# OnurBasci/TransformerBasedNavierStokeSolver

Measured on AMD Instinct MI355X. Metric: ns64_train_samples_per_s, higher is better.
Workload: dtype f32

## Files before the change

transformerbasednavierstokesolver_amd/csrc/pa2d_gemm.hip:

```cpp
#include "pa2d_gemm_common.h"
#include <string.h>


static Pa2dEnv read_env() {
    auto is = [](const char* n, const char* pre) { const char* e = getenv(n); return e && strncmp(e, pre, strlen(pre)) == 0; };
    auto num = [](const char* n, int dflt) { const char* e = getenv(n); return (e && e[0]) ? atoi(e) : dflt; };
    Pa2dEnv v;
    v.conv_halo = is("PA2D_CONV_HALO", "o") ? 0 : (is("PA2D_CONV_HALO", "f") ? 2 : 1);
    v.mc_big_off = is("PA2D_MC_BIG", "o") ? 1 : 0;
    v.kc_bk16 = num("PA2D_KC_BK", 0) == 16 ? 1 : 0;
    v.mc_bk = num("PA2D_MC_BK", 16) == 32 ? 32 : 16;
    v.mc_splits = num("PA2D_MC_SPLITS", 0);
    v.mcb_splits = num("PA2D_MCB_SPLITS", 0);
    v.lin_dw_split = is("PA2D_LIN_DW_SPLIT", "of") ? 0 : 1;
    v.lin_panel = is("PA2D_LIN_PANEL", "of") ? 0 : 1;
    v.lin_rowpanel = is("PA2D_LIN_ROWPANEL", "of") ? 0 : 1;
    v.lin_small_split = is("PA2D_LIN_SMALL_SPLIT", "of") ? 0 : 1;
    v.conv_mfma16 = num("PA2D_CONV_MFMA", 16) == 32 ? 0 : 1;
    v.mc_mfma16 = num("PA2D_MC_MFMA", 16) == 32 ? 0 : 1;
    v.split_big = num("PA2D_SPLIT_BIG", 1);
    v.slice_map = is("PA2D_SLICE_MAP", "l") ? 0 : 1;
    v.default_engine = is("PA2D_GEMM", "f") ? 0 : (is("PA2D_GEMM", "b") ? 2 : 1);
    return v;
}
static Pa2dEnv g_env = read_env();
const Pa2dEnv& pa2d_env() { return g_env; }
static int kc_bk(bool im2col, int Cin) {
    if (im2col && pa2d_env().kc_bk16) return 16;
    return (!im2col || (Cin % 32) == 0) ? 32 : 16;
}
KCTile kc_tile(int M, int N, bool im2col, int Cin) {
    const int tiles_m = ceil_div(M, 128);
    const long long t128 = (long long)tiles_m * ceil_div(N, 128);
    const long long t12864 = (long long)tiles_m * ceil_div(N, 64);
    const int bk = kc_bk(im2col, Cin);
    if (N > 64 && t128 >= 384) return {128, 128, bk};
    if (t12864 >= 384 || M <= 64) return {128, 64, bk};
    return {64, 64, bk};
}
bool use_split(int engine, int N, bool im2col, int Cin) {
    const int m = engine;
    if (m == 1) return im2col && N > 64 && (Cin % 32) == 0;
    if (m == 2) return N > 64 && (!im2col || (Cin % 32) == 0);
    return false;
}

int launch_kc(const KCParams& p_in, bool im2col, hipStream_t st, hipEvent_t ev0, hipEvent_t ev1) {
    KCParams p = p_in;
    if (!engine_ok(p.engine)) return PA2D_ERR_ARG;
    if (p.M <= 0 || p.N <= 0 || p.K <= 0) return PA2D_OK;
    if (!p.bias2) p.bias_split = 0x7fffffff;
    {
// ... 18 lines not shown
        if (p.wsrc) {
            rc = launch_pack_weight_image(p.wsrc, p.wsn, p.wsk, p.wimg, p.N, p.K, st);
            if (rc) return rc;
        }
        KCParams pp = p;
        pp.M = p.M - p.M % 128;
        rc = launch_kc_rowpanel(pp, p.wimg, st);
        if (!rc && pp.M < p.M) {
            KCParams pt = p_in;
            pt.wimg = nullptr;
            pt.M = p.M - pp.M;
            pt.A = p.A + (size_t)pp.M * p.lda;
            pt.C = p.C + (size_t)pp.M * p.ldc;
            if (p.res) pt.res = p.res + (size_t)pp.M * p.ldres;
            if (p.aux) pt.aux = p.aux + (size_t)pp.M * p.ldaux;
            rc = launch_kc(pt, false, st);
        }
    } else if (panel_applies(p, im2col)) {
        KCParams pp = p;
        pp.M = p.M - p.M % 256;
        rc = launch_kc_panel(pp, st);
        if (!rc && pp.M < p.M) {
            KCParams pt = p_in;
            const size_t ea = p.io_bf16 ? 2 : 4, es = p.io_bf16 ? 2 : 4;
            pt.M = p.M - pp.M;
            pt.A = (const float*)((const char*)p.A + (size_t)pp.M * p.lda * ea);
            pt.C = (float*)((char*)p.C + (size_t)pp.M * p.ldc * es);
            if (p.res) pt.res = (const float*)((const char*)p.res + (size_t)pp.M * p.ldres * es);
            if (p.aux) pt.aux = (float*)((char*)p.aux + (size_t)pp.M * p.ldaux * es);
            rc = launch_kc(pt, false, st);
        }
    } else if (p.io_bf16 || use_split(p.engine, p.N, im2col, p.Cin)) rc = launch_kc_split(p, im2col, st);
    else if (kc_split_small_applies(p, im2col)) rc = launch_kc_split_small(p, st);
    else rc = launch_kc_f32(p, im2col, kc_tile(p.M, p.N, im2col, p.Cin), st);
    if (rc) return rc;
    if (ev1 && hipEventRecord(ev1, st) != hipSuccess) return PA2D_ERR_ARG;
    return PA2D_OK;
}

template <int TAPS>
__global__ void repack_kernel(const float* __restrict__ w0, const float* __restrict__ w1, float* __restrict__ dst,
                              int mode, int N, int K, int C, int Cin, int NK) {
    const long long idx = (long long)blockIdx.x * blockDim.x + threadIdx.x;
    if (mode == 0) {
        if (idx >= (long long)N * K) return;
        const int n = (int)(idx % N), k = (int)(idx / N);
        dst[idx] = w0[(size_t)n * K + k];
    } else if (mode == 1) {
        if (idx >= (long long)NK * C * TAPS * Cin) return;
        const int CH = K;
        const int c16 = (int)(idx % CH);
        const int tap = (int)((idx / CH) % TAPS);
        const int cic = (int)((idx / (TAPS * CH)) % (Cin / CH));
        const int co = (int)(idx / ((long long)Cin * TAPS));
        const int ci = cic * CH + c16;
        const float* src = co < C ? w0 : w1;
        dst[idx] = src[((size_t)(co % C) * Cin + ci) * TAPS + tap];
    } else {
        if (idx >= (long long)NK * C * TAPS * Cin) return;
        const int CH = K;
        const int c16 = (int)(idx % CH);
        const int tap = (int)((idx / CH) % TAPS);
        const int cic = (int)((idx / (TAPS * CH)) % (NK * C / CH));
        const int ci = (int)(idx / ((long long)NK * C * TAPS));
        const int co = cic * CH + c16;
        const float* src = co < C ? w0 : w1;
// ... 62 lines not shown
                           const void* wimg, void* ws, size_t ws_bytes, int M, int N, int K, int act, int engine,
                           hipStream_t st) {
    KCParams p = dense_fwd_params(x, ldx, w, ldw, bias, res, ldres, y, ldy, pre, ldpre, M, N, K, act, engine, false);
    const size_t img = rowpanel_image_bytes(N, K, engine);
    if (img && wimg) p.wimg = const_cast<void*>(wimg);
    else if (ws && img && ws_bytes >= img) { p.wimg = ws; p.wsrc = w; p.wsn = ldw; p.wsk = 1; }
    return launch_kc(p, false, st);
}

int pa2d_gemm_bwd_data(const float* dy, long long lddy, const float* w, long long ldw, const float* pre,
                       long long ldpre, int act, float* dx, long long lddx, const void* wimg, void* ws, size_t ws_bytes, int M,
                       int N, int K, int engine, hipStream_t st) {
    if (ldw != K) return PA2D_ERR_ARG;
    if (N & 3) return PA2D_ERR_ARG;
    if (M <= 0) return PA2D_OK;
    if (ws_bytes < (size_t)N * K * sizeof(float)) return PA2D_ERR_WORKSPACE;
    float* const wt_ws = (float*)ws;
    KCParams p = dense_bwd_data_params(dy, lddy, wt_ws, pre, ldpre, act, dx, lddx, M, N, K, engine, false);
    const size_t img = rowpanel_image_bytes(K, N, engine);
    if (img && wimg) p.wimg = const_cast<void*>(wimg);
    else if (img && ws_bytes >= (size_t)N * K * sizeof(float) + img) {
        p.wimg = (char*)ws + (size_t)N * K * sizeof(float); p.wsrc = w; p.wsn = 1; p.wsk = ldw;
    }
    if (!(p.wimg && rowpanel_applies(p) && (M % 128) == 0)) {
        const int rc = launch_repack(w, nullptr, wt_ws, 0, N, K, 0, 0, st);
        if (rc) return rc;
    }
    return launch_kc(p, false, st);
}

size_t pa2d_gemm_bwd_weight_workspace(int M, int N, int K, int engine) {
    (void)engine;
    const MCPlan pl = plan_mc(N, K, M);
    return (pl.slab_floats + (size_t)pl.splits * N) * sizeof(float);
}

int pa2d_gemm_bwd_weight(const float* dy, long long lddy, const float* x, long long ldx, float* dw, float* db,
                         void* ws, size_t ws_bytes, int M, int N, int K, int accumulate, int engine, hipStream_t st) {
    if (!engine_ok(engine)) return PA2D_ERR_ARG;
    if (M <= 0) {
        if (accumulate) return PA2D_OK;
        const int rz = pa2d_zero(dw, sizeof(float) * N * K, st);
        return rz ? rz : pa2d_zero(db, sizeof(float) * N, st);
    }
    if (ws_bytes < pa2d_gemm_bwd_weight_workspace(M, N, K, engine)) return PA2D_ERR_WORKSPACE;
    const MCPlan pl = plan_mc(N, K, M);
    float* cs = db ? (float*)ws + pl.slab_floats : nullptr;
    const bool bfk = (engine == 1 || engine == 2) && pl.big && mc_f32src_applies(N, K, M, lddy, ldx);
    int rc = bfk ? launch_mc_f32src(dy, lddy, N, x, ldx, K, M, (float*)ws, pl, engine == 2 ? 1 : 3, cs, st)
                 : launch_mc(dy, lddy, N, x, ldx, K, M, false, 0, 0, 0, (float*)ws, pl, engine, st, cs);
    if (rc) return rc;
    rc = launch_reduce((const float*)ws, pl.splits, (long long)N * K, dw, nullptr, 0, 0, 0, st, accumulate);
    if (rc) return rc;
    if (db) rc = launch_reduce(cs, pl.splits, N, db, nullptr, 0, 0, 0, st, accumulate);
    return rc;
}


int pa2d_gemm_bias_act_fwd_bf16(const void* x, long long ldx, const float* w, long long ldw, const float* bias,
                                const void* res, long long ldres, void* y, long long ldy, void* pre, long long ldpre,
                                int M, int N, int K, int act, hipStream_t st) {
    return launch_kc(dense_fwd_params(x, ldx, w, ldw, bias, res, ldres, y, ldy, pre, ldpre, M, N, K, act, 2, true), false, st);
}

int pa2d_gemm_bwd_data_bf16(const void* dy, long long lddy, const float* w, long long ldw, const void* pre,
                            long long ldpre, int act, void* dx, long long lddx, float* wt_ws, int M, int N, int K,
                            hipStream_t st) {
    if (ldw != K) return PA2D_ERR_ARG;
    if (N & 3) return PA2D_ERR_ARG;
    if (M <= 0) return PA2D_OK;
    int rc = launch_repack(w, nullptr, wt_ws, 0, N, K, 0, 0, st);
    if (rc) return rc;
    return launch_kc(dense_bwd_data_params(dy, lddy, wt_ws, pre, ldpre, act, dx, lddx, M, N, K, 2, true), false, st);
}

size_t pa2d_gemm_bwd_weight_workspace_bf16(int M, int N, int K) {
    const MCPlan pl = plan_mc_planes_big(N, K, M);
    size_t a = pl.slab_floats, b = (size_t)colsum_blocks(M) * N;
// ... 24 lines not shown
```

transformerbasednavierstokesolver_amd/csrc/pa2d_gemm_common.h:

```cpp
#pragma once
#include "pa2d_internal.h"
#include "pa2d_bf16_split.h"
#include <stdlib.h>

#define EPI_ACT 1
#define EPI_STORE_PRE 2
#define EPI_MUL_DACT 4

struct KCParams {
    const float* A; long long lda;
    const float* B; long long ldb;
    float* C; long long ldc;
    const float* bias;
    const float* bias2; int bias_split;
    int depth;
    const float* res; long long ldres;
    float* aux; long long ldaux;
    int M, N, K;
    int act, epi;
    int H, W, Cin;
    unsigned a_bytes, b_bytes;
    unsigned c_bytes, res_bytes, aux_bytes;
    int apre;
    int engine;
// ... 104 lines not shown
bool kc_split_small_applies(const KCParams& p, bool im2col);
int launch_kc_split_small(const KCParams& p, hipStream_t st);
size_t planes_bytes(long long rows, int C, int NT);
int launch_split_planes(const float* src, long long ld, void* dst, long long rows, int C, int NT, hipStream_t st);
int launch_repack_split(const float* w0, const float* w1, void* dst, int bwd, int NT, int C, int Cin, hipStream_t st,
                        int taps = 9);
bool panel_applies(const KCParams& p, bool im2col);
int launch_kc_panel(const KCParams& p, hipStream_t st);
size_t rowpanel_image_bytes(int N, int K, int engine);
bool rowpanel_applies(const KCParams& p);
int launch_pack_weight_image(const float* w, long long sn, long long sk, void* img, int N, int K, hipStream_t st);
int launch_kc_rowpanel(const KCParams& p, const void* img, hipStream_t st);
bool conv_halo_applies(const KCParams& p);
int launch_conv_halo(const KCParams& p, hipStream_t st);
MCPlan plan_mc(int Mi, int Nj, int Mk);
int launch_mc(const float* A, long long lda, int Mi, const float* B, long long ldb, int Nj, int Mk, bool im2col,
              int H, int W, int Cin, float* slab, const MCPlan& pl, int engine, hipStream_t st, float* colsum = nullptr,
              int taps = 9, int depth = 1);
int launch_reduce(const float* slab, int nslab, long long count, float* out, float* out2, int mode, int C, int Cin,
                  hipStream_t st, int accumulate = 0, int taps = 9);
int pa2d_launch_reduce(const float* slab, int nslab, long long count, float* out, hipStream_t st);
bool mc_planes_supported(int C, int Cin);
int launch_mc_planes(const void* PA, const void* PB, int C, int Cin, int Mk, int H, int W, float* slab,
                     const MCPlan& pl, int NT, hipStream_t st);
bool mc_planes_big_applies(int C, int Cin, int Mk);
MCPlan plan_mc_planes_big(int Mi, int Nj, int Mk);
int launch_mc_planes_big(const void* PA, const void* PB, int C, int Cin, int Mk, int H, int W, float* slab,
                         const MCPlan& pl, int NT, hipStream_t st);
int launch_mc_planes_big_raw(const void* PA, int Mi, const void* PB, int Cin, int taps, int Mk, int H, int W, float* slab,
                             const MCPlan& pl, int NT, hipStream_t st);
bool mc_f32src_applies(int Mi, int Nj, int Mk, long long lda, long long ldb);
int launch_mc_f32src(const float* A, long long lda, int Mi, const float* B, long long ldb, int Nj, int Mk, float* slab,
                     const MCPlan& pl, int NT, float* colsum, hipStream_t st);
int colsum_blocks(int M);
int launch_colsum_bf16(const void* X, long long ld, int M, int N, float* out, float* partial, hipStream_t st,
                       float* out2 = nullptr, int split = 0, int accumulate = 0);
int launch_colsum(const float* X, long long ld, int M, int N, float* out, float* partial, hipStream_t st,
                  float* out2 = nullptr, int split = 0, int accumulate = 0);
```

transformerbasednavierstokesolver_amd/csrc/pa2d_gemm_mc_planes.hip:

```cpp
#include "pa2d_gemm_common.h"
#include "pa2d_bf16_split.h"

struct MCPlanesParams {
    const void* PA; int chA;
    const void* PB; int chB;
    float* slab;
    int Mi, Nj, Mk, chunks_per_split, splits, H, W, Cin;
    unsigned a_bytes, b_bytes;
    int taps;
    long long lda, ldb;
    float* colsum;
};

__device__ __forceinline__ unsigned img_off(int row, int ch) {
    return 256u * row + 16u * (ch ^ (((row & 3) << 2) | ((row >> 2) & 3)));
}

template <int NT, int KS, bool F32SRC = false, bool MF16 = false>
__global__ __launch_bounds__(256, 2) void gemm_mc_planes_kernel(const MCPlanesParams p) {
    constexpr int PIMG = 4096;
    constexpr int STAGE = 2 * NT * KS * PIMG;
    constexpr int NP = 2 * NT * KS;
    __shared__ __attribute__((aligned(16))) unsigned char smem[(MF16 ? 3 : 2) * STAGE];

    const int tid = threadIdx.x, lane = tid & 63, wave = tid >> 6;
    const int tiles_i = (p.Mi + 127) / 128, tiles_j = (p.Nj + 127) / 128;
    int tj, ti, split;
    {
        const int tiles = tiles_i * tiles_j;
        if ((p.splits & 7) == 0) {
            const int xcd = blockIdx.x & 7, slot = blockIdx.x >> 3, q = p.splits >> 3;
            split = xcd * q + slot / tiles;
            const int t = slot % tiles;
            tj = t % tiles_j;
            ti = t / tiles_j;
        } else {
            tj = blockIdx.x % tiles_j;
            ti = (blockIdx.x / tiles_j) % tiles_i;
            split = blockIdx.x / tiles;
        }
    }
    const int wm = wave >> 1, wn = wave & 1;
    const int total_chunks = (p.Mk + 15) / 16;
    const int c_begin = split * p.chunks_per_split;
    const int c_end = min(total_chunks, c_begin + p.chunks_per_split);

    const int j0 = tj * 128, tap = j0 / p.Cin, cb0 = (j0 - tap * p.Cin) >> 5, ca0 = (ti * 128) >> 5;
    const int tap_dy = tap / 3 - 1, tap_dx = tap - (tap / 3) * 3 - 1, tap_shift = tap_dy * p.W + tap_dx;
    const int HW = p.H * p.W;

    const __amdgpu_buffer_rsrc_t ra_rsrc = __builtin_amdgcn_make_buffer_rsrc(const_cast<void*>(p.PA), 0, p.a_bytes, 0x00020000);
    const __amdgpu_buffer_rsrc_t rb_rsrc = __builtin_amdgcn_make_buffer_rsrc(const_cast<void*>(p.PB), 0, p.b_bytes, 0x00020000);

    int s_row[NP];
    unsigned s_goff[NP], s_lds[NP];
    bool s_isb[NP];
// ... 94 lines not shown
        __builtin_amdgcn_ds_read_tr16_b64_v4i16((lds_s16x4*)(smem + ((base_[0] ^ ((unsigned)(t_) << 5)) + (pl_) * PIMG))), \
        __builtin_amdgcn_ds_read_tr16_b64_v4i16((lds_s16x4*)(smem + ((base_[1] ^ ((unsigned)(t_) << 5)) + (pl_) * PIMG))), \
        0, 1, 2, 3, 4, 5, 6, 7))
#define MP16_MMA(ib_, AF)                                                                                 \
    _Pragma("unroll") for (int j = 0; j < 4; ++j) {        \
        acc[ib_][j] = __builtin_amdgcn_mfma_f32_16x16x32_bf16(xf[j][1], AF[1], acc[ib_][j], 0, 0, 0);     \
        acc[ib_][j] = __builtin_amdgcn_mfma_f32_16x16x32_bf16(xf[j][0], AF[2], acc[ib_][j], 0, 0, 0);     \
        acc[ib_][j] = __builtin_amdgcn_mfma_f32_16x16x32_bf16(xf[j][2], AF[0], acc[ib_][j], 0, 0, 0);     \
        acc[ib_][j] = __builtin_amdgcn_mfma_f32_16x16x32_bf16(xf[j][0], AF[1], acc[ib_][j], 0, 0, 0);     \
        acc[ib_][j] = __builtin_amdgcn_mfma_f32_16x16x32_bf16(xf[j][1], AF[0], acc[ib_][j], 0, 0, 0);     \
        acc[ib_][j] = __builtin_amdgcn_mfma_f32_16x16x32_bf16(xf[j][0], AF[0], acc[ib_][j], 0, 0, 0);     \
    }
        bf16x8 pk[2][NT];
#define MP16_CONVERT()                                                                                    \
    _Pragma("unroll") for (int op = 0; op < 2; ++op) {                                                    \
        const u32x4 u0_ = rg[op * 2], u1_ = rg[op * 2 + 1];                                               \
        const float4 v0_ = make_float4(__uint_as_float(u0_.x), __uint_as_float(u0_.y), __uint_as_float(u0_.z), __uint_as_float(u0_.w)); \
        const float4 v1_ = make_float4(__uint_as_float(u1_.x), __uint_as_float(u1_.y), __uint_as_float(u1_.z), __uint_as_float(u1_.w)); \
        if (op == 0 && do_cs) {                                                                           \
            cs[0] += v0_.x; cs[1] += v0_.y; cs[2] += v0_.z; cs[3] += v0_.w;                               \
            cs[4] += v1_.x; cs[5] += v1_.y; cs[6] += v1_.z; cs[7] += v1_.w;                               \
        }                                                                                                 \
        bf16x4 h0_, m0_, l0_, h1_, m1_, l1_;                                                              \
        split3(v0_, h0_, m0_, l0_);                                                                       \
        split3(v1_, h1_, m1_, l1_);                                                                       \
        pk[op][0] = __builtin_shufflevector(h0_, h1_, 0, 1, 2, 3, 4, 5, 6, 7);                            \
        pk[op][1] = __builtin_shufflevector(m0_, m1_, 0, 1, 2, 3, 4, 5, 6, 7);                            \
        pk[op][2] = __builtin_shufflevector(l0_, l1_, 0, 1, 2, 3, 4, 5, 6, 7);                            \
    }
#define MP16_WRITE(buf_)                                                                                  \
    _Pragma("unroll") for (int op = 0; op < 2; ++op) _Pragma("unroll") for (int pl = 0; pl < NT; ++pl)    \
        *reinterpret_cast<bf16x8*>(smem + (buf_) * STAGE + flds + (op * NT + pl) * PIMG) = pk[op][pl];
        const int nst = c_end - c_begin, steps = (nst + 1) >> 1;
        if (nst > 0) {
            MP_LOAD(c_begin)
            MP16_CONVERT()
            MP16_WRITE(0)
            MP_LOAD(c_begin + 1)
            MP16_CONVERT()
            MP16_WRITE(1)
            if (steps > 1) { MP_LOAD(c_begin + 2) }
        }
        __syncthreads();
        int sp = 0, sq = 1, sr = 2;
        for (int k = 0; k < steps; ++k) {
            const bool has_next = k + 1 < steps;
            const unsigned lo = (unsigned)((kq >> 1) ? sq : sp) * (unsigned)STAGE;
            const unsigned ua[2] = {fa[0] + lo, fa[1] + lo};
            const unsigned ub[2] = {fb[0] + lo + NT * PIMG, fb[1] + lo + NT * PIMG};
            bf16x8 xf[4][NT];
#pragma unroll
            for (int j = 0; j < 4; ++j)
#pragma unroll
                for (int pl = 0; pl < NT; ++pl) xf[j][pl] = MP16_FRAG(ub, j, pl);
            bf16x8 afc[NT], afn[NT];
#pragma unroll
            for (int pl = 0; pl < NT; ++pl) afc[pl] = MP16_FRAG(ua, 0, pl);
#pragma unroll
            for (int ib = 0; ib < 4; ++ib) {
                if (ib < 3) {
#pragma unroll
                    for (int pl = 0; pl < NT; ++pl) afn[pl] = MP16_FRAG(ua, ib + 1, pl);
                }
                if (ib == 1 && has_next) {
                    MP16_CONVERT()
                    MP16_WRITE(sr)
                    MP_LOAD(c_begin + 2 * k + 3)
                }
                if (ib == 3) {
                    if (has_next) {
                        MP16_CONVERT()
                        if (k + 2 < steps) { MP_LOAD(c_begin + 2 * k + 4) }
                    }
                    __syncthreads();
                    if (has_next) { MP16_WRITE(sp) }
                }
                MP16_MMA(ib, afc)
#pragma unroll
                for (int pl = 0; pl < NT; ++pl) afc[pl] = afn[pl];
            }
            __syncthreads();
            const int t = sp;
            sp = sr;
            sr = sq;
            sq = t;
        }
#undef MP16_CONVERT
#undef MP16_WRITE
#undef MP16_MMA
#undef MP16_FRAG
        if (do_cs) {
            float* sm = reinterpret_cast<float*>(smem);
#pragma unroll
            for (int e = 0; e < 8; ++e) sm[frow * 128 + fc8 * 8 + e] = cs[e];
            __syncthreads();
            if (tid < 128) {
                float t = 0.f;
#pragma unroll
                for (int r = 0; r < 16; ++r) t += sm[r * 128 + tid];
                if (ti * 128 + tid < p.Mi) p.colsum[(size_t)split * p.Mi + ti * 128 + tid] = t;
            }
        }
        float* out = p.slab + (size_t)split * p.Mi * p.Nj;
#pragma unroll
        for (int j = 0; j < 4; ++j) {
            const int col = tj * 128 + wn * 64 + j * 16 + 4 * kq;
#pragma unroll
            for (int ib = 0; ib < 4; ++ib) {
                const int row = ti * 128 + wm * 64 + ib * 16 + (lane & 15);
                if (row < p.Mi && col < p.Nj) *reinterpret_cast<f32x4*>(out + (size_t)row * p.Nj + col) = acc[ib][j];
            }
        }
        return;
    }

    f32x16 acc[2][2];
#pragma unroll
    for (int i = 0; i < 2; ++i)
// ... 415 lines not shown
            hipError_t e = hipFuncSetAttribute(reinterpret_cast<const void*>(&gemm_mc_planes_big_kernel<3, 1>),
                                               hipFuncAttributeMaxDynamicSharedMemorySize, smem);
            if (e != hipSuccess) return (int)e;
        }
        hipLaunchKernelGGL((gemm_mc_planes_big_kernel<3, 1>), grid, dim3(512), smem, st, p, per_xcd);
    } else {
        const int smem = 2 * 2 * 1 * 4 * 8192;
        {
            hipError_t e = hipFuncSetAttribute(reinterpret_cast<const void*>(&gemm_mc_planes_big_kernel<1, 4>),
                                               hipFuncAttributeMaxDynamicSharedMemorySize, smem);
            if (e != hipSuccess) return (int)e;
        }
        hipLaunchKernelGGL((gemm_mc_planes_big_kernel<1, 4>), grid, dim3(512), smem, st, p, per_xcd);
    }
    PA2D_CHECK_LAUNCH();
    return PA2D_OK;
}

bool mc_f32src_applies(int Mi, int Nj, int Mk, long long lda, long long ldb) {
    return pa2d_env().lin_dw_split && (Mi % 8) == 0 && (Nj % 8) == 0 && Mi > 64 && Nj > 64 && Mk >= 16 * 8 * 16 && (lda % 4) == 0 && (ldb % 4) == 0;
}

int launch_mc_f32src(const float* A, long long lda, int Mi, const float* B, long long ldb, int Nj, int Mk, float* slab,
                     const MCPlan& pl, int NT, float* colsum, hipStream_t st) {
    if (!pl.big) return PA2D_ERR_UNSUPPORTED;
    MCPlanesParams p = {};
    p.PA = A; p.PB = B; p.slab = slab; p.lda = lda; p.ldb = ldb; p.colsum = colsum;
    p.Mi = Mi; p.Nj = Nj; p.Mk = Mk; p.chunks_per_split = pl.chunks_per_split; p.splits = pl.splits;
    p.H = 1; p.W = 1; p.Cin = Nj; p.taps = 1; p.chA = 0; p.chB = 0;
    const unsigned long long ab = ((unsigned long long)(Mk - 1) * lda + Mi) * 4ull, bb = ((unsigned long long)(Mk - 1) * ldb + Nj) * 4ull;
    if (ab >= 0xFFFFFFF0ull || bb >= 0xFFFFFFF0ull) return PA2D_ERR_UNSUPPORTED;
    p.a_bytes = (unsigned)ab; p.b_bytes = (unsigned)bb;
    const dim3 grid(ceil_div(Mi, 128) * ceil_div(Nj, 128) * pl.splits);
    if (NT == 3 && pa2d_env().mc_mfma16 && (Nj % 4) == 0 && (reinterpret_cast<uintptr_t>(slab) & 15) == 0)
        hipLaunchKernelGGL((gemm_mc_planes_kernel<3, 1, true, true>), grid, dim3(256), 0, st, p);
    else if (NT == 3) hipLaunchKernelGGL((gemm_mc_planes_kernel<3, 1, true>), grid, dim3(256), 0, st, p);
    else hipLaunchKernelGGL((gemm_mc_planes_kernel<1, 4, true>), grid, dim3(256), 0, st, p);
    PA2D_CHECK_LAUNCH();
    return PA2D_OK;
}
```

transformerbasednavierstokesolver_amd/csrc/pa2d_internal.h:

```cpp
#pragma once
#include <hip/hip_runtime.h>
#include <stdint.h>

typedef float f32x16 __attribute__((ext_vector_type(16)));
typedef float f32x4 __attribute__((ext_vector_type(4)));

#define PA2D_OK 0
#define PA2D_ERR_ARG 1001
#define PA2D_ERR_UNSUPPORTED 1002
#define PA2D_ERR_WORKSPACE 1003

#define PA2D_CHECK_LAUNCH()                         \
    do {                                            \
        hipError_t e__ = hipGetLastError();         \
        if (e__ != hipSuccess) return (int)e__;     \
    } while (0)

enum { ACT_NONE = 0, ACT_GELU = 1, ACT_TANH = 2, ACT_SIGMOID = 3, ACT_RELU = 4, ACT_SOFTPLUS = 5,
       ACT_ELU = 6, ACT_SILU = 7 };

__device__ __forceinline__ float normal_cdf(float x, float& e_out) {
#pragma clang fp contract(off)
    const float z = fabsf(x) * 0.70710678118654752440f;
    const float t = __builtin_amdgcn_rcpf(fmaf(0.3275911f, z, 1.0f));
// ... 67 lines not shown
}


__device__ __forceinline__ float buf_load1(__amdgpu_buffer_rsrc_t r, unsigned voff) {
    return __uint_as_float(__builtin_amdgcn_raw_buffer_load_b32(r, voff, 0, 0));
}
__device__ __forceinline__ void buf_store1(__amdgpu_buffer_rsrc_t r, unsigned voff, float v) {
    __builtin_amdgcn_raw_buffer_store_b32(__float_as_uint(v), r, voff, 0, 0);
}

__device__ __forceinline__ float2 buf_load2(__amdgpu_buffer_rsrc_t r, unsigned voff) {
    typedef unsigned int u32x2_ __attribute__((ext_vector_type(2)));
    const u32x2_ v = __builtin_amdgcn_raw_buffer_load_b64(r, voff, 0, 0);
    return make_float2(__uint_as_float(v.x), __uint_as_float(v.y));
}
__device__ __forceinline__ void buf_store4(__amdgpu_buffer_rsrc_t r, unsigned voff, float4 v) {
    u32x4 u = {__float_as_uint(v.x), __float_as_uint(v.y), __float_as_uint(v.z), __float_as_uint(v.w)};
    __builtin_amdgcn_raw_buffer_store_b128(u, r, voff, 0, 0);
}

#define PA2D_ACT_SAVE_DERIVATIVE_BIT 0x100

struct Pa2dEnv {
    int conv_halo;
    int mc_big_off;
    int kc_bk16;
    int mc_bk;
    int mc_splits;
    int mcb_splits;
    int lin_dw_split;
    int lin_panel;
    int conv_mfma16;
    int mc_mfma16;
    int lin_small_split;
    int lin_rowpanel;
    int split_big;
    int slice_map;
    int default_engine;
};
const Pa2dEnv& pa2d_env();

static inline int pa2d_zero(void* p, size_t bytes, hipStream_t st) {
    if (!p || !bytes) return PA2D_OK;
    return (int)hipMemsetAsync(p, 0, bytes, st);
}
static inline int ceil_div(int a, int b) { return (a + b - 1) / b; }
static inline long long ceil_div_ll(long long a, long long b) { return (a + b - 1) / b; }

struct ReduceSegs { int nseg; long long begin[5]; float* dst[4]; };
int pa2d_launch_reduce_segs(const float* slab, int nslab, long long count, const ReduceSegs& segs, int accumulate,
                            hipStream_t st);

typedef __bf16 bf16_t;
template <typename T> struct Act;
template <> struct Act<float> {
    static constexpr unsigned ES = 4;
    static __device__ __forceinline__ float4 ld4(const float* p) { return *reinterpret_cast<const float4*>(p); }
    static __device__ __forceinline__ void st4(float* p, float4 v) { *reinterpret_cast<float4*>(p) = v; }
    static __device__ __forceinline__ float ld1(const float* p) { return *p; }
    static __device__ __forceinline__ float4 bld4(__amdgpu_buffer_rsrc_t r, unsigned off) { return buf_load4(r, off); }
    static __device__ __forceinline__ float2 bld2(__amdgpu_buffer_rsrc_t r, unsigned off) { return buf_load2(r, off); }
    static __device__ __forceinline__ float bld1(__amdgpu_buffer_rsrc_t r, unsigned off) { return buf_load1(r, off); }
    static __device__ __forceinline__ float bld1s(__amdgpu_buffer_rsrc_t r, unsigned off, unsigned soff) {
        return __uint_as_float(__builtin_amdgcn_raw_buffer_load_b32(r, off, soff, 0));
    }
    static __device__ __forceinline__ void bst4(__amdgpu_buffer_rsrc_t r, unsigned off, float4 v) { buf_store4(r, off, v); }
// ... 72 lines not shown
```

Baseline: 69.11.

## Add skinny-K CUDA-core GEMM paths and two-slot MFMA16 weight-grad pipeline

Adds dedicated kernels for linear layers with tiny inner dimension (K or Nj ≤ 16): a forward kernel that keeps a 4-column weight slice in registers and streams rows, and a weight-gradient kernel that accumulates per-block partials in registers, reduces them in shared memory and writes records for a later reduce. Both are on by default and replace tiled MFMA GEMMs that waste work on such narrow shapes. Also adds an optional two-slot shared-memory variant of the MFMA16 f32-source weight-grad kernel with higher occupancy, selected only by an environment variable. The risks are enlarged workspace sizing and plain FMA throughput when a shape matches but is large.

```diff
diff --git a/transformerbasednavierstokesolver_amd/csrc/pa2d_gemm.hip b/transformerbasednavierstokesolver_amd/csrc/pa2d_gemm.hip
--- a/transformerbasednavierstokesolver_amd/csrc/pa2d_gemm.hip
+++ b/transformerbasednavierstokesolver_amd/csrc/pa2d_gemm.hip
@@ -18,6 +18,8 @@
     v.lin_small_split = is("PA2D_LIN_SMALL_SPLIT", "of") ? 0 : 1;
     v.conv_mfma16 = num("PA2D_CONV_MFMA", 16) == 32 ? 0 : 1;
     v.mc_mfma16 = num("PA2D_MC_MFMA", 16) == 32 ? 0 : 1;
+    v.mc_lin_slots = is("PA2D_MC_MFMA", "16x2") ? 2 : 3;
+    v.lin_skinny = is("PA2D_LIN_SKINNY", "of") ? 0 : 1;
     v.split_big = num("PA2D_SPLIT_BIG", 1);
     v.slice_map = is("PA2D_SLICE_MAP", "l") ? 0 : 1;
     v.default_engine = is("PA2D_GEMM", "f") ? 0 : (is("PA2D_GEMM", "b") ? 2 : 1);
@@ -102,6 +104,7 @@
         }
     } else if (p.io_bf16 || use_split(p.engine, p.N, im2col, p.Cin)) rc = launch_kc_split(p, im2col, st);
     else if (kc_split_small_applies(p, im2col)) rc = launch_kc_split_small(p, st);
+    else if (skinny_fwd_applies(p, im2col)) rc = launch_skinny_fwd(p, st);
     else rc = launch_kc_f32(p, im2col, kc_tile(p.M, p.N, im2col, p.Cin), st);
     if (rc) return rc;
     if (ev1 && hipEventRecord(ev1, st) != hipSuccess) return PA2D_ERR_ARG;
@@ -230,7 +233,12 @@
 size_t pa2d_gemm_bwd_weight_workspace(int M, int N, int K, int engine) {
     (void)engine;
     const MCPlan pl = plan_mc(N, K, M);
-    return (pl.slab_floats + (size_t)pl.splits * N) * sizeof(float);
+    size_t fl = pl.slab_floats + (size_t)pl.splits * N;
+    if (skinny_wgrad_shape(N, K)) {
+        const size_t sk = skinny_wgrad_ws_floats(N, K, M);
+        if (sk > fl) fl = sk;
+    }
+    return fl * sizeof(float);
 }
 
 int pa2d_gemm_bwd_weight(const float* dy, long long lddy, const float* x, long long ldx, float* dw, float* db,
@@ -242,6 +250,15 @@
         return rz ? rz : pa2d_zero(db, sizeof(float) * N, st);
     }
     if (ws_bytes < pa2d_gemm_bwd_weight_workspace(M, N, K, engine)) return PA2D_ERR_WORKSPACE;
+    if (skinny_wgrad_applies(dy, lddy, N, x, ldx, K, ws)) {
+        int nrec;
+        float* csk;
+        int rs = launch_skinny_wgrad(dy, lddy, N, x, ldx, K, M, (float*)ws, db != nullptr, nrec, csk, st);
+        if (rs) return rs;
+        rs = launch_reduce((const float*)ws, nrec, (long long)N * K, dw, nullptr, 0, 0, 0, st, accumulate);
+        if (rs) return rs;
+        return db ? launch_reduce(csk, nrec, N, db, nullptr, 0, 0, 0, st, accumulate) : PA2D_OK;
+    }
     const MCPlan pl = plan_mc(N, K, M);
     float* cs = db ? (float*)ws + pl.slab_floats : nullptr;
     const bool bfk = (engine == 1 || engine == 2) && pl.big && mc_f32src_applies(N, K, M, lddy, ldx);
diff --git a/transformerbasednavierstokesolver_amd/csrc/pa2d_gemm_common.h b/transformerbasednavierstokesolver_amd/csrc/pa2d_gemm_common.h
--- a/transformerbasednavierstokesolver_amd/csrc/pa2d_gemm_common.h
+++ b/transformerbasednavierstokesolver_amd/csrc/pa2d_gemm_common.h
@@ -160,6 +160,13 @@
 bool mc_f32src_applies(int Mi, int Nj, int Mk, long long lda, long long ldb);
 int launch_mc_f32src(const float* A, long long lda, int Mi, const float* B, long long ldb, int Nj, int Mk, float* slab,
                      const MCPlan& pl, int NT, float* colsum, hipStream_t st);
+bool skinny_fwd_applies(const KCParams& p, bool im2col);
+int launch_skinny_fwd(const KCParams& p, hipStream_t st);
+bool skinny_wgrad_shape(int Mi, int Nj);
+size_t skinny_wgrad_ws_floats(int Mi, int Nj, int Mk);
+bool skinny_wgrad_applies(const float* dY, long long lddy, int Mi, const float* X, long long ldx, int Nj, const void* ws);
+int launch_skinny_wgrad(const float* dY, long long lddy, int Mi, const float* X, long long ldx, int Nj, int Mk, float* ws,
+                        bool want_colsum, int& nrec, float*& colsum_out, hipStream_t st);
 int colsum_blocks(int M);
 int launch_colsum_bf16(const void* X, long long ld, int M, int N, float* out, float* partial, hipStream_t st,
                        float* out2 = nullptr, int split = 0, int accumulate = 0);
diff --git a/transformerbasednavierstokesolver_amd/csrc/pa2d_gemm_mc_planes.hip b/transformerbasednavierstokesolver_amd/csrc/pa2d_gemm_mc_planes.hip
--- a/transformerbasednavierstokesolver_amd/csrc/pa2d_gemm_mc_planes.hip
+++ b/transformerbasednavierstokesolver_amd/csrc/pa2d_gemm_mc_planes.hip
@@ -16,12 +16,12 @@
     return 256u * row + 16u * (ch ^ (((row & 3) << 2) | ((row >> 2) & 3)));
 }
 
-template <int NT, int KS, bool F32SRC = false, bool MF16 = false>
-__global__ __launch_bounds__(256, 2) void gemm_mc_planes_kernel(const MCPlanesParams p) {
+template <int NT, int KS, bool F32SRC = false, bool MF16 = false, int SLOTS = 3>
+__global__ __launch_bounds__(256, (MF16 && SLOTS == 2) ? 3 : 2) void gemm_mc_planes_kernel(const MCPlanesParams p) {
     constexpr int PIMG = 4096;
     constexpr int STAGE = 2 * NT * KS * PIMG;
     constexpr int NP = 2 * NT * KS;
-    __shared__ __attribute__((aligned(16))) unsigned char smem[(MF16 ? 3 : 2) * STAGE];
+    __shared__ __attribute__((aligned(16))) unsigned char smem[(MF16 ? SLOTS : 2) * STAGE];
 
     const int tid = threadIdx.x, lane = tid & 63, wave = tid >> 6;
     const int tiles_i = (p.Mi + 127) / 128, tiles_j = (p.Nj + 127) / 128;
@@ -182,6 +182,97 @@
     _Pragma("unroll") for (int op = 0; op < 2; ++op) _Pragma("unroll") for (int pl = 0; pl < NT; ++pl)    \
         *reinterpret_cast<bf16x8*>(smem + (buf_) * STAGE + flds + (op * NT + pl) * PIMG) = pk[op][pl];
         const int nst = c_end - c_begin, steps = (nst + 1) >> 1;
+        if constexpr (SLOTS == 2) {
+#define MP2_LOAD(op_, c_)                                                                                 \
+    _Pragma("unroll") for (int s = 0; s < 2; ++s) {                                                       \
+        const int m_ = ((c_) + s) * 16 + frow;                                                            \
+        const bool ok_ = m_ < p.Mk && (c_) + s < c_end && ((op_) ? fok_b : fok_a);       \
+        const unsigned o_ = ok_ ? (unsigned)m_ * ((op_) ? fpitch_b : fpitch_a) + ((op_) ? fcol_b : fcol_a) : OOB_OFF; \
+        rg[2 * s] = __builtin_amdgcn_raw_buffer_load_b128((op_) ? rb_rsrc : ra_rsrc, o_, 0, 0);           \
+        rg[2 * s + 1] = __builtin_amdgcn_raw_buffer_load_b128((op_) ? rb_rsrc : ra_rsrc, o_ == OOB_OFF ? OOB_OFF : o_ + 16u, 0, 0); \
+    }
+#define MP2_CONVERT(op_)                                                                                  \
+    _Pragma("unroll") for (int s = 0; s < 2; ++s) {                                                       \
+        const u32x4 u0_ = rg[2 * s], u1_ = rg[2 * s + 1];                                                 \
+        const float4 v0_ = make_float4(__uint_as_float(u0_.x), __uint_as_float(u0_.y), __uint_as_float(u0_.z), __uint_as_float(u0_.w)); \
+        const float4 v1_ = make_float4(__uint_as_float(u1_.x), __uint_as_float(u1_.y), __uint_as_float(u1_.z), __uint_as_float(u1_.w)); \
+        if ((op_) == 0 && do_cs) {                                                                        \
+            cs[0] += v0_.x; cs[1] += v0_.y; cs[2] += v0_.z; cs[3] += v0_.w;                               \
+            cs[4] += v1_.x; cs[5] += v1_.y; cs[6] += v1_.z; cs[7] += v1_.w;                               \
+        }                                                                                                 \
+        bf16x4 h0_, m0_, l0_, h1_, m1_, l1_;                                                              \
+        split3(v0_, h0_, m0_, l0_);                                                                       \
+        split3(v1_, h1_, m1_, l1_);                                                                       \
+        pk[s][0] = __builtin_shufflevector(h0_, h1_, 0, 1, 2, 3, 4, 5, 6, 7);                             \
+        pk[s][1] = __builtin_shufflevector(m0_, m1_, 0, 1, 2, 3, 4, 5, 6, 7);                             \
+        pk[s][2] = __builtin_shufflevector(l0_, l1_, 0, 1, 2, 3, 4, 5, 6, 7);                             \
+    }
+#define MP2_WRITE(op_)                                                                                    \
+    _Pragma("unroll") for (int s = 0; s < 2; ++s) _Pragma("unroll") for (int pl = 0; pl < NT; ++pl)       \
+        *reinterpret_cast<bf16x8*>(smem + s * STAGE + flds + ((op_) * NT + pl) * PIMG) = pk[s][pl];
+#define MP2_MMA(ib_, AF, j0_)                                                                             \
+    _Pragma("unroll") for (int jj = 0; jj < 2; ++jj) {                \
+        acc[ib_][(j0_) + jj] = __builtin_amdgcn_mfma_f32_16x16x32_bf16(xf[jj][1], AF[1], acc[ib_][(j0_) + jj], 0, 0, 0); \
+        acc[ib_][(j0_) + jj] = __builtin_amdgcn_mfma_f32_16x16x32_bf16(xf[jj][0], AF[2], acc[ib_][(j0_) + jj], 0, 0, 0); \
+        acc[ib_][(j0_) + jj] = __builtin_amdgcn_mfma_f32_16x16x32_bf16(xf[jj][2], AF[0], acc[ib_][(j0_) + jj], 0, 0, 0); \
+        acc[ib_][(j0_) + jj] = __builtin_amdgcn_mfma_f32_16x16x32_bf16(xf[jj][0], AF[1], acc[ib_][(j0_) + jj], 0, 0, 0); \
+        acc[ib_][(j0_) + jj] = __builtin_amdgcn_mfma_f32_16x16x32_bf16(xf[jj][1], AF[0], acc[ib_][(j0_) + jj], 0, 0, 0); \
+        acc[ib_][(j0_) + jj] = __builtin_amdgcn_mfma_f32_16x16x32_bf16(xf[jj][0], AF[0], acc[ib_][(j0_) + jj], 0, 0, 0); \
+    }
+            const unsigned lo = (unsigned)(kq >> 1) * (unsigned)STAGE;
+            unsigned ua[2] = {fa[0] + lo, fa[1] + lo};
+            unsigned ub[2] = {fb[0] + lo + NT * PIMG, fb[1] + lo + NT * PIMG};
+            if (nst > 0) {
+                MP2_LOAD(0, c_begin)
+                MP2_CONVERT(0)
+                MP2_WRITE(0)
+                MP2_LOAD(1, c_begin)
+                MP2_CONVERT(1)
+                MP2_WRITE(1)
+                if (steps > 1) { MP2_LOAD(1, c_begin + 2) }
+            }
+            __syncthreads();
+            for (int k = 0; k < steps; ++k) {
+                const bool has_next = k + 1 < steps;
+#pragma unroll
+                for (int h = 0; h < 2; ++h) {
+                    asm volatile("" : "+v"(ua[0]), "+v"(ua[1]), "+v"(ub[0]), "+v"(ub[1]));
+                    bf16x8 xf[2][NT];
+#pragma unroll
+                    for (int jj = 0; jj < 2; ++jj)
+#pragma unroll
+                        for (int pl = 0; pl < NT; ++pl) xf[jj][pl] = MP16_FRAG(ub, 2 * h + jj, pl);
+                    if (h == 1) {
+                        __syncthreads();
+                        if (has_next) {
+                            MP2_WRITE(1)
+                            MP2_LOAD(0, c_begin + 2 * k + 2)
+                        }
+                    }
+#pragma unroll
+                    for (int ib = 0; ib < 4; ++ib) {
+                        if (h == 0 && ib == 2 && has_next) { MP2_CONVERT(1) }
+                        if (h == 1 && ib == 3 && has_next) { MP2_CONVERT(0) }
+                        bf16x8 af[NT];
+#pragma unroll
+                        for (int pl = 0; pl < NT; ++pl) af[pl] = MP16_FRAG(ua, ib, pl);
+                        if (h == 1 && ib == 3) {
+                            __syncthreads();
+                            if (has_next) {
+                                MP2_WRITE(0)
+                                if (k + 2 < steps) { MP2_LOAD(1, c_begin + 2 * k + 4) }
+                            }
+                        }
+                        MP2_MMA(ib, af, 2 * h)
+                    }
+                }
+                __syncthreads();
+            }
+#undef MP2_LOAD
+#undef MP2_CONVERT
+#undef MP2_WRITE
+#undef MP2_MMA
+        } else {
         if (nst > 0) {
             MP_LOAD(c_begin)
             MP16_CONVERT()
@@ -234,6 +325,7 @@
             sp = sr;
             sr = sq;
             sq = t;
+        }
         }
 #undef MP16_CONVERT
 #undef MP16_WRITE
@@ -715,8 +807,10 @@
     if (ab >= 0xFFFFFFF0ull || bb >= 0xFFFFFFF0ull) return PA2D_ERR_UNSUPPORTED;
     p.a_bytes = (unsigned)ab; p.b_bytes = (unsigned)bb;
     const dim3 grid(ceil_div(Mi, 128) * ceil_div(Nj, 128) * pl.splits);
-    if (NT == 3 && pa2d_env().mc_mfma16 && (Nj % 4) == 0 && (reinterpret_cast<uintptr_t>(slab) & 15) == 0)
-        hipLaunchKernelGGL((gemm_mc_planes_kernel<3, 1, true, true>), grid, dim3(256), 0, st, p);
+    const bool mf16 = NT == 3 && pa2d_env().mc_mfma16 && (Nj % 4) == 0 && (reinterpret_cast<uintptr_t>(slab) & 15) == 0;
+    if (mf16 && pa2d_env().mc_lin_slots == 2)
+        hipLaunchKernelGGL((gemm_mc_planes_kernel<3, 1, true, true, 2>), grid, dim3(256), 0, st, p);
+    else if (mf16) hipLaunchKernelGGL((gemm_mc_planes_kernel<3, 1, true, true, 3>), grid, dim3(256), 0, st, p);
     else if (NT == 3) hipLaunchKernelGGL((gemm_mc_planes_kernel<3, 1, true>), grid, dim3(256), 0, st, p);
     else hipLaunchKernelGGL((gemm_mc_planes_kernel<1, 4, true>), grid, dim3(256), 0, st, p);
     PA2D_CHECK_LAUNCH();
diff --git a/transformerbasednavierstokesolver_amd/csrc/pa2d_gemm_skinny.hip b/transformerbasednavierstokesolver_amd/csrc/pa2d_gemm_skinny.hip
--- /dev/null
+++ b/transformerbasednavierstokesolver_amd/csrc/pa2d_gemm_skinny.hip
@@ -0,0 +1,194 @@
+#include "pa2d_gemm_common.h"
+
+static inline int pow2_shift_ge(int n, int max_shift) {
+    int s = 0;
+    while ((1 << s) < n && s < max_shift) ++s;
+    return s;
+}
+static inline bool al16(const void* p) { return (reinterpret_cast<uintptr_t>(p) & 15) == 0; }
+
+template <int K, int EPI>
+__global__ __launch_bounds__(256) void skinny_fwd_kernel(const KCParams p, const int qshift, const int rows_per_wg) {
+    const int tid = threadIdx.x, qw = 1 << qshift;
+    const int q = blockIdx.y * qw + (tid & (qw - 1)), rl = tid >> qshift, rp = 256 >> qshift;
+    if (4 * q >= p.N) return;
+    float w[4][K];
+#pragma unroll
+    for (int c = 0; c < 4; ++c)
+#pragma unroll
+        for (int k4 = 0; k4 < K / 4; ++k4) {
+            const float4 t = *reinterpret_cast<const float4*>(p.B + (size_t)(4 * q + c) * p.ldb + 4 * k4);
+            w[c][4 * k4] = t.x; w[c][4 * k4 + 1] = t.y; w[c][4 * k4 + 2] = t.z; w[c][4 * k4 + 3] = t.w;
+        }
+    const float4 b = p.bias ? *reinterpret_cast<const float4*>(p.bias + 4 * q) : make_float4(0.f, 0.f, 0.f, 0.f);
+    const int r0 = blockIdx.x * rows_per_wg, r1 = min(p.M, r0 + rows_per_wg);
+    const bool st_aux = EPI == 1 || (EPI == 2 && (p.epi & EPI_STORE_PRE));
+    const bool do_act = EPI == 1 || (EPI == 2 && (p.epi & EPI_ACT));
+#pragma unroll 2
+    for (int r = r0 + rl; r < r1; r += rp) {
+        float x[K];
+#pragma unroll
+        for (int k4 = 0; k4 < K / 4; ++k4) {
+            const float4 t = *reinterpret_cast<const float4*>(p.A + (size_t)r * p.lda + 4 * k4);
+            x[4 * k4] = t.x; x[4 * k4 + 1] = t.y; x[4 * k4 + 2] = t.z; x[4 * k4 + 3] = t.w;
+        }
+        float v[4] = {0.f, 0.f, 0.f, 0.f};
+#pragma unroll
+        for (int k = 0; k < K; ++k)
+#pragma unroll
+            for (int c = 0; c < 4; ++c) v[c] = fmaf(x[k], w[c][k], v[c]);
+        v[0] += b.x; v[1] += b.y; v[2] += b.z; v[3] += b.w;
+        float o[4], a[4];
+#pragma unroll
+        for (int c = 0; c < 4; ++c) {
+            if (EPI == 1) {
+                a[c] = p.aux_deriv ? dgelu_f(v[c]) : v[c];
+                o[c] = gelu_f(v[c]);
+            } else if (EPI == 2) {
+                a[c] = p.aux_deriv ? act_bwd(p.act, v[c]) : v[c];
+                o[c] = do_act ? act_fwd(p.act, v[c]) : v[c];
+            } else {
+                a[c] = o[c] = v[c];
+            }
+        }
+        if (st_aux) *reinterpret_cast<float4*>(p.aux + (size_t)r * p.ldaux + 4 * q) = make_float4(a[0], a[1], a[2], a[3]);
+        *reinterpret_cast<float4*>(p.C + (size_t)r * p.ldc + 4 * q) = make_float4(o[0], o[1], o[2], o[3]);
+    }
+}
+
+bool skinny_fwd_applies(const KCParams& p, bool im2col) {
+    if (!pa2d_env().lin_skinny || im2col || p.io_bf16) return false;
+    if (p.K > 16 || (p.K & 3) || (p.N & 3) || p.res || p.bias2 || (p.epi & EPI_MUL_DACT)) return false;
+    if ((p.epi & EPI_STORE_PRE) && (!p.aux || (p.ldaux & 3) || !al16(p.aux))) return false;
+    return !(p.lda & 3) && !(p.ldb & 3) && !(p.ldc & 3) && al16(p.A) && al16(p.B) && al16(p.C) && (!p.bias || al16(p.bias));
+}
+
+template <int K>
+static void skinny_fwd_launch(const KCParams& p, int epi, dim3 grid, int qshift, int rows_per_wg, hipStream_t st) {
+    if (epi == 0) hipLaunchKernelGGL((skinny_fwd_kernel<K, 0>), grid, dim3(256), 0, st, p, qshift, rows_per_wg);
+    else if (epi == 1) hipLaunchKernelGGL((skinny_fwd_kernel<K, 1>), grid, dim3(256), 0, st, p, qshift, rows_per_wg);
+    else hipLaunchKernelGGL((skinny_fwd_kernel<K, 2>), grid, dim3(256), 0, st, p, qshift, rows_per_wg);
+}
+
+int launch_skinny_fwd(const KCParams& p, hipStream_t st) {
+    const int nq = p.N / 4;
+    const int qshift = pow2_shift_ge(nq, 8), rp = 256 >> qshift;
+    long long gx = ceil_div_ll(p.M, (long long)rp * 16);
+    if (gx > 4096) gx = 4096;
+    int rows_per_wg = (int)ceil_div_ll(p.M, gx);
+    rows_per_wg = ceil_div(rows_per_wg, rp) * rp;
+    const dim3 grid((unsigned)ceil_div(p.M, rows_per_wg), (unsigned)ceil_div(nq, 1 << qshift));
+    const int epi = p.epi == 0 ? 0 : ((p.epi == (EPI_ACT | EPI_STORE_PRE) && p.act == ACT_GELU) ? 1 : 2);
+    switch (p.K) {
+        case 4: skinny_fwd_launch<4>(p, epi, grid, qshift, rows_per_wg, st); break;
+        case 8: skinny_fwd_launch<8>(p, epi, grid, qshift, rows_per_wg, st); break;
+        case 12: skinny_fwd_launch<12>(p, epi, grid, qshift, rows_per_wg, st); break;
+        case 16: skinny_fwd_launch<16>(p, epi, grid, qshift, rows_per_wg, st); break;
+        default: return PA2D_ERR_UNSUPPORTED;
+    }
+    PA2D_CHECK_LAUNCH();
+    return PA2D_OK;
+}
+
+struct SkinnyWgradParams {
+    const float* dY; long long lddy; int Mi;
+    const float* X; long long ldx; int Mk;
+    int rows_per_wg, qshift;
+    float* rec;
+    float* colsum;
+};
+
+template <int NJ>
+__global__ __launch_bounds__(512) void skinny_wgrad_kernel(const SkinnyWgradParams p) {
+    __shared__ float4 red[512];
+    const int tid = threadIdx.x, qw = 1 << p.qshift;
+    const int ql = tid & (qw - 1), q = blockIdx.y * qw + ql, rl = tid >> p.qshift, nrl = 512 >> p.qshift;
+    const bool active = 4 * q < p.Mi;
+    float acc[4][NJ];
+    float cs[4] = {0.f, 0.f, 0.f, 0.f};
+#pragma unroll
+    for (int c = 0; c < 4; ++c)
+#pragma unroll
+        for (int j = 0; j < NJ; ++j) acc[c][j] = 0.f;
+    const int r0 = blockIdx.x * p.rows_per_wg, r1 = min(p.Mk, r0 + p.rows_per_wg);
+    if (active) {
+#pragma unroll 2
+        for (int r = r0 + rl; r < r1; r += nrl) {
+            const float4 d = *reinterpret_cast<const float4*>(p.dY + (size_t)r * p.lddy + 4 * q);
+            float x[NJ];
+#pragma unroll
+            for (int j4 = 0; j4 < NJ / 4; ++j4) {
+                const float4 t = *reinterpret_cast<const float4*>(p.X + (size_t)r * p.ldx + 4 * j4);
+                x[4 * j4] = t.x; x[4 * j4 + 1] = t.y; x[4 * j4 + 2] = t.z; x[4 * j4 + 3] = t.w;
+            }
+            const float dv[4] = {d.x, d.y, d.z, d.w};
+#pragma unroll
+            for (int c = 0; c < 4; ++c) {
+                cs[c] += dv[c];
+#pragma unroll
+                for (int j = 0; j < NJ; ++j) acc[c][j] = fmaf(dv[c], x[j], acc[c][j]);
+            }
+        }
+    }
+    float* const rec = p.rec + (size_t)blockIdx.x * p.Mi * NJ;
+#pragma unroll
+    for (int pass = 0; pass <= NJ; ++pass) {
+        const int c = pass / (NJ / 4), j4 = pass % (NJ / 4);
+        float4 v = pass < NJ ? make_float4(acc[c % 4][4 * j4], acc[c % 4][4 * j4 + 1], acc[c % 4][4 * j4 + 2], acc[c % 4][4 * j4 + 3])
+                             : make_float4(cs[0], cs[1], cs[2], cs[3]);
+        if (nrl > 1) {
+            red[tid] = v;
+            __syncthreads();
+            if (rl == 0)
+                for (int l = 1; l < nrl; ++l) {
+                    const float4 t = red[l * qw + ql];
+                    v.x += t.x; v.y += t.y; v.z += t.z; v.w += t.w;
+                }
+        }
+        if (rl == 0 && active) {
+            if (pass < NJ) *reinterpret_cast<float4*>(rec + (size_t)(4 * q + c) * NJ + 4 * j4) = v;
+            else if (p.colsum) *reinterpret_cast<float4*>(p.colsum + (size_t)blockIdx.x * p.Mi + 4 * q) = v;
+        }
+        if (nrl > 1) __syncthreads();
+    }
+}
+
+static int skinny_wgrad_plan(int Mi, int Mk, int& qshift, int& rows_per_wg) {
+    qshift = pow2_shift_ge(Mi / 4, 9);
+    const int nrl = 512 >> qshift;
+    if (Mk < 1) Mk = 1;
+    rows_per_wg = ceil_div(Mk, 512);
+    if (rows_per_wg < nrl * 8) rows_per_wg = nrl * 8;
+    rows_per_wg = ceil_div(rows_per_wg, nrl) * nrl;
+    return ceil_div(Mk, rows_per_wg);
+}
+
+bool skinny_wgrad_shape(int Mi, int Nj) { return pa2d_env().lin_skinny && Nj <= 16 && Nj > 0 && !(Nj & 3) && Mi > 0 && !(Mi & 3); }
+
+size_t skinny_wgrad_ws_floats(int Mi, int Nj, int Mk) {
+    int qs, rpw;
+    return (size_t)skinny_wgrad_plan(Mi, Mk, qs, rpw) * ((size_t)Mi * Nj + Mi);
+}
+
+bool skinny_wgrad_applies(const float* dY, long long lddy, int Mi, const float* X, long long ldx, int Nj, const void* ws) {
+    return skinny_wgrad_shape(Mi, Nj) && !(lddy & 3) && !(ldx & 3) && al16(dY) && al16(X) && al16(ws);
+}
+
+int launch_skinny_wgrad(const float* dY, long long lddy, int Mi, const float* X, long long ldx, int Nj, int Mk, float* ws,
+                        bool want_colsum, int& nrec, float*& colsum_out, hipStream_t st) {
+    SkinnyWgradParams p;
+    p.dY = dY; p.lddy = lddy; p.Mi = Mi; p.X = X; p.ldx = ldx; p.Mk = Mk;
+    nrec = skinny_wgrad_plan(Mi, Mk, p.qshift, p.rows_per_wg);
+    p.rec = ws;
+    p.colsum = colsum_out = want_colsum ? ws + (size_t)nrec * Mi * Nj : nullptr;
+    const dim3 grid((unsigned)nrec, (unsigned)ceil_div(Mi / 4, 1 << p.qshift));
+    switch (Nj) {
+        case 4: hipLaunchKernelGGL((skinny_wgrad_kernel<4>), grid, dim3(512), 0, st, p); break;
+        case 8: hipLaunchKernelGGL((skinny_wgrad_kernel<8>), grid, dim3(512), 0, st, p); break;
+        case 12: hipLaunchKernelGGL((skinny_wgrad_kernel<12>), grid, dim3(512), 0, st, p); break;
+        case 16: hipLaunchKernelGGL((skinny_wgrad_kernel<16>), grid, dim3(512), 0, st, p); break;
+        default: return PA2D_ERR_UNSUPPORTED;
+    }
+    PA2D_CHECK_LAUNCH();
+    return PA2D_OK;
+}
diff --git a/transformerbasednavierstokesolver_amd/csrc/pa2d_internal.h b/transformerbasednavierstokesolver_amd/csrc/pa2d_internal.h
--- a/transformerbasednavierstokesolver_amd/csrc/pa2d_internal.h
+++ b/transformerbasednavierstokesolver_amd/csrc/pa2d_internal.h
@@ -123,6 +123,8 @@
     int lin_panel;
     int conv_mfma16;
     int mc_mfma16;
+    int mc_lin_slots;
+    int lin_skinny;
     int lin_small_split;
     int lin_rowpanel;
     int split_big;
```

Result: no change. 68.88 (-0.3%).
